# tzt101/MichiGAN

Measured on NVIDIA H100. Metric: 512x512 images/sec (generator forward), higher is better.
Workload: dtype fp16/bf16 tensor-core operands (bf16 hi+lo split where needed), fp32 accumulate and storage

## Files before the change

michigan_b200/csrc/mg_conv3x3.cu:

```cuda
#include <cuda.h>
#include <cuda_runtime.h>
#include <cstring>
#include <type_traits>
#include "mg_ptx.cuh"
#include "mg_internal.h"
#include "mg_epilogue.cuh"

namespace mg {

constexpr int kGM = 2;
constexpr int kPatchW = 8 * kGM + 2;
constexpr int kPatchH = 16 + 2;
constexpr int kPatchTx = kPatchW * kPatchH * 128;
constexpr int kPatchBytes = (kPatchTx + 1023) & ~1023;
constexpr int kMaxBSlots = 8;
constexpr int kASlots = 2;

struct Conv3Params {
    IgemmParams g;
    int groups_w, num_groups, b_slots, b_slot_bytes, steps_hi, steps_lo, n_items, bar3_off;
};

template <int FMT, int BN, bool MERGED, int SPEC, int CW, bool REG>
__global__ void __launch_bounds__(kThreads, 1)
conv3x3_group_kernel(const __grid_constant__ CUtensorMap tmA, const __grid_constant__ CUtensorMap tmA2,
                     const __grid_constant__ CUtensorMap tmB, const Conv3Params q) {
    constexpr int kAcc = MERGED ? 2 * BN : BN;
    const IgemmParams& p = q.g;
    extern __shared__ __align__(1024) uint8_t smem_raw[];
    uint8_t* smem = reinterpret_cast<uint8_t*>((reinterpret_cast<uintptr_t>(smem_raw) + 1023) & ~uintptr_t(1023));
    uint8_t* a_ring = smem;
    uint8_t* b_ring = smem + kASlots * kPatchBytes;
    uint64_t* bars = reinterpret_cast<uint64_t*>(smem + q.bar3_off);
    uint64_t* bfull = bars;
    uint64_t* bempty = bars + kMaxBSlots;
    uint64_t* afull = bars + 2 * kMaxBSlots;
    uint64_t* aempty = afull + kASlots;
    float* acc_tile = reinterpret_cast<float*>(smem + p.acc_off);

    const int warp = threadIdx.x >> 5;
    const int lane = threadIdx.x & 31;

    if (warp == kNumEpiWarps && lane == 0) {
        tma_prefetch_desc(&tmA);
        tma_prefetch_desc(&tmA2);
        tma_prefetch_desc(&tmB);
        for (int s = 0; s < q.b_slots; ++s) { mbar_init(&bfull[s], 1); mbar_init(&bempty[s], kNumEpiWarps); }
        for (int s = 0; s < kASlots; ++s) { mbar_init(&afull[s], 1); mbar_init(&aempty[s], kNumEpiWarps); }
        fence_barrier_init();
    }
    __syncthreads();
    const int groups_per_img = q.groups_w * p.tiles_h;
    const bool split = p.parts > 1;

    if (warp >= kNumEpiWarps) {
        setmaxnreg_dec<kProducerRegs>();
        if (warp == kNumEpiWarps && lane == 0) {
            int bs = 0, as_ = 0;
            uint32_t bph = 0, aphs = 0;
            int gia = blockIdx.x, ita = 0;
            long long a_issued = 0, item = 0;
            auto issue_a = [&](bool must) -> bool {
                if (gia >= q.num_groups) return false;
                if (!must && !mbar_test_wait(&aempty[as_], aphs ^ 1)) return false;
                if (must) mbar_wait_report(&aempty[as_], aphs ^ 1);
                const int mga = gia / p.n_tiles;
                const int gwa = mga % q.groups_w, tha = (mga / q.groups_w) % p.tiles_h, tna = mga / groups_per_img;
                const int kca = split ? (ita >> 1) : ita, parta = split ? (ita & 1) : 0;
                mbar_arrive_expect_tx(&afull[as_], (uint32_t)kPatchTx);
                tma_load_4d(a_ring + (size_t)as_ * kPatchBytes, parta ? &tmA2 : &tmA, &afull[as_], kca * p.kelem, gwa * (8 * kGM) - 1,
                            tha * 16 - 1, tna);
                if (++as_ == kASlots) { as_ = 0; aphs ^= 1; }
                if (++ita == q.n_items) { ita = 0; gia += gridDim.x; }
                ++a_issued;
                return true;
            };
            for (int gi = blockIdx.x; gi < q.num_groups; gi += gridDim.x) {
                const int nt = gi % p.n_tiles;
                for (int it = 0; it < q.n_items; ++it, ++item) {
                    const int kc = split ? (it >> 1) : it, part = split ? (it & 1) : 0;
                    if (a_issued <= item) issue_a(true);
                    const int steps = part ? q.steps_lo : q.steps_hi;
                    for (int st = 0; st < steps; ++st) {
                        if (a_issued < item + kASlots) issue_a(false);
                        int tap, wsel;
                        if (steps == 18) { tap = st >> 1; wsel = st & 1; } else { tap = st; wsel = 0; }
                        const int kofs = (split ? (tap * 2 + wsel) : tap) * p.Cin + kc * p.kelem;
                        mbar_wait_report(&bempty[bs], bph ^ 1);
                        uint8_t* sb = b_ring + (size_t)bs * q.b_slot_bytes;
                        if (p.merged && part == 0) {
                            mbar_arrive_expect_tx(&bfull[bs], (uint32_t)(2 * p.BN * 128));
                            tma_load_2d(sb, &tmB, &bfull[bs], kofs, nt * p.BN);
                            tma_load_2d(sb + p.BN * 128, &tmB, &bfull[bs], kofs + p.Cin, nt * p.BN);
                        } else {
                            mbar_arrive_expect_tx(&bfull[bs], (uint32_t)(p.BN * 128));
                            tma_load_2d(sb, &tmB, &bfull[bs], kofs, nt * p.BN);
                        }
                        if (++bs == q.b_slots) { bs = 0; bph ^= 1; }
                    }
                }
            }
        }
    } else {
        setmaxnreg_inc<kConsumerRegs>();
        const int wg = warp >> 2;
        const int quarter = warp & 3;
        const int half = warp >> 2;
        const uint32_t a_base0 = smem_u32(a_ring), b_base0 = smem_u32(b_ring);
        float acc0[kAcc / 2], acc1[kAcc / 2];
        int bs = 0, as_ = 0;
        uint32_t bph = 0, aphs = 0;
        int held_b = -1, held_a = -1;
        auto release_held = [&]() {
            __syncwarp();
            if (lane == 0) {
                if (held_b >= 0) mbar_arrive(&bempty[held_b]);
                if (held_a >= 0) mbar_arrive(&aempty[held_a]);
            }
            held_b = held_a = -1;
        };
        for (int gi = blockIdx.x; gi < q.num_groups; gi += gridDim.x) {
            const int nt = gi % p.n_tiles;
            const int mg = gi / p.n_tiles;
            const int gw = mg % q.groups_w, th = (mg / q.groups_w) % p.tiles_h, tn = mg / groups_per_img;
            for (int it = 0; it < q.n_items; ++it) {
                const int part = split ? (it & 1) : 0;
                mbar_wait(&afull[as_], aphs);
                const uint32_t a_base = a_base0 + (uint32_t)(as_ * kPatchBytes) + (uint32_t)(wg * 8 * kPatchW * 128);
                const int steps = part ? q.steps_lo : q.steps_hi;
                auto item = [&](auto n_cols) {
                    constexpr int N = decltype(n_cols)::value;
                    for (int st = 0; st < steps; ++st) {
                        const int tap = steps == 18 ? (st >> 1) : st;
                        const int kh = tap / 3, kw = tap - kh * 3;
                        mbar_wait(&bfull[bs], bph);
                        const uint32_t a_tap = a_base + (uint32_t)((kh * kPatchW + kw) * 128);
                        const uint64_t db = wg_desc_sw128(b_base0 + (uint32_t)(bs * q.b_slot_bytes), 1024);
                        wgmma_fence();
#pragma unroll
                        for (int k = 0; k < 4; ++k) {
                            const uint32_t accum = (it | st | k) != 0 ? 1u : 0u;
                            const uint64_t da0 = wg_desc_sw128(a_tap + (uint32_t)(k * 32), (uint32_t)(kPatchW * 128));
                            const uint64_t da1 = wg_desc_sw128(a_tap + (uint32_t)(8 * 128 + k * 32), (uint32_t)(kPatchW * 128));
                            wgmma_step<FMT, N>(acc0, da0, db + (uint64_t)(2 * k), accum);
                            wgmma_step<FMT, N>(acc1, da1, db + (uint64_t)(2 * k), accum);
                        }
                        wgmma_commit();
                        wgmma_wait<1>();
                        release_held();
                        held_b = bs;
                        if (++bs == q.b_slots) { bs = 0; bph ^= 1; }
                    }
                };
                if (MERGED && part == 1) item(std::integral_constant<int, BN>{});
                else item(std::integral_constant<int, kAcc>{});
                held_a = as_;
                if (++as_ == kASlots) { as_ = 0; aphs ^= 1; }
            }
            wgmma_wait<0>();
            wgmma_fence_operand(acc0);
            wgmma_fence_operand(acc1);
            release_held();
            if constexpr (REG) {
                epilogue_frag<SPEC, BN, MERGED>(p, acc0, acc1, nt, gw * kGM, th, tn, wg, quarter, lane);
            } else {
                float* scr = reinterpret_cast<float*>(smem + p.epi_off) + warp * (32 * (CW + 4));
                bar_sync(1, kNumEpiWarps * 32);
                acc_store(acc_tile, p.acc_ld, acc0, kAcc, wg * 64);
                bar_sync(1, kNumEpiWarps * 32);
                epilogue_tile<SPEC, CW>(p, scr, acc_tile, nt, gw * kGM, th, tn, quarter, half, lane);
                bar_sync(1, kNumEpiWarps * 32);
                acc_store(acc_tile, p.acc_ld, acc1, kAcc, wg * 64);
                bar_sync(1, kNumEpiWarps * 32);
                epilogue_tile<SPEC, CW>(p, scr, acc_tile, nt, gw * kGM + 1, th, tn, quarter, half, lane);
            }
        }
    }
}

constexpr bool conv3_reg_epilogue(int bn, bool merged, int spec) { return !(bn == 128 && !merged && spec == 0); }

struct Conv3Launch {
    const CUtensorMap *tmA, *tmA2, *tmB;
    const Conv3Params* q;
    int grid;
    size_t smem_bytes;
    cudaStream_t stream;
    bool reg;
    template <int FMT, int BN, bool MERGED, int SPEC, int CW>
    int run() const {
        if constexpr (conv_variant_exists<FMT, BN, MERGED, SPEC, CW>()) {
            if constexpr (CW == 16 && conv3_reg_epilogue(BN, MERGED, SPEC)) {
                if (reg) {
                    static thread_local int attr_dev_reg = -1;
                    return launch_conv_kernel(conv3x3_group_kernel<FMT, BN, MERGED, SPEC, CW, true>, attr_dev_reg, grid, smem_bytes,
                                              stream, *tmA, *tmA2, *tmB, *q);
                }
            }
            static thread_local int attr_dev = -1;
            return launch_conv_kernel(conv3x3_group_kernel<FMT, BN, MERGED, SPEC, CW, false>, attr_dev, grid, smem_bytes, stream, *tmA,
                                      *tmA2, *tmB, *q);
        } else {
            return set_error(-14, "conv3x3: no kernel variant for format %d, BN %d, merged %d, SPEC %d, CW %d", FMT, BN, (int)MERGED,
                             SPEC, CW);
        }
    }
};

int conv3x3_group_launch(const mg_igemm_args* a, IgemmParams& p, int BN, int cw, int scratch_bytes, int spec, cudaStream_t stream) {
    if (!(a->KH == 3 && a->KW == 3 && a->stride == 1 && p.pad_h == 1 && p.pad_w == 1 && a->H == a->OH && a->W == a->OW && p.epi_impl == 1 &&
          a->OW >= 16 && a->OW % 16 == 0 && a->OH >= 16 && p.os == 1))
        return 0;
    const bool reg = tune(TK_EPI_REG) != 0 && conv3_reg_epilogue(BN, p.merged != 0, spec);
    if (reg) { scratch_bytes = 0; cw = 16; }
    const int acc_bytes = reg ? 0 : 128 * p.acc_ld * 4;
    {
        const int avail0 = 227 * 1024 - 1024 - 512 - scratch_bytes - acc_bytes - kASlots * kPatchBytes;
        if (avail0 / (p.acc_cols * 128) < 3) return 0;
    }
    Conv3Params q;
    memset(&q, 0, sizeof(q));
    p.TW = 8; p.TH = 16; p.TN = 1;
    p.tiles_w = a->OW / 8;
    p.tiles_h = (a->OH + 15) / 16;
    p.tiles_n = a->N;
    p.num_tiles = p.tiles_w * p.tiles_h * p.tiles_n * p.n_tiles;
    p.halo = 0;
    q.groups_w = p.tiles_w / kGM;
    q.num_groups = q.groups_w * p.tiles_h * p.tiles_n * p.n_tiles;
    const bool split = a->split != 0;
    q.steps_hi = (split && !p.merged) ? 18 : 9;
    q.steps_lo = 9;
    q.n_items = p.kchunks * (split ? 2 : 1);
    q.b_slot_bytes = p.acc_cols * 128;
    const int avail = 227 * 1024 - 1024 - 512 - scratch_bytes - acc_bytes - kASlots * kPatchBytes;
    q.b_slots = avail / q.b_slot_bytes;
    if (q.b_slots > kMaxBSlots) q.b_slots = kMaxBSlots;
    const size_t ring_bytes = (size_t)kASlots * kPatchBytes + (size_t)q.b_slots * q.b_slot_bytes;
    q.bar3_off = (int)ring_bytes;
    p.epi_off = (int)ring_bytes + 512;
    p.acc_off = p.epi_off + scratch_bytes;
    p.parts = p.merged ? 2 : (split ? 3 : 1);
    q.g = p;

    CUtensorMap tmA, tmA2, tmB;
    const int kelem = p.kelem;
    const int esz = a->a_fmt == 0 ? 4 : 2;
    const CUtensorMapDataType dt = a->a_fmt == 0 ? CU_TENSOR_MAP_DATA_TYPE_FLOAT32
                                 : a->a_fmt == 1 ? CU_TENSOR_MAP_DATA_TYPE_FLOAT16 : CU_TENSOR_MAP_DATA_TYPE_BFLOAT16;
    {
        cuuint64_t dims[4] = {(cuuint64_t)a->Cin, (cuuint64_t)a->W, (cuuint64_t)a->H, (cuuint64_t)a->N};
        cuuint64_t strides[3] = {(cuuint64_t)a->Cin * esz, (cuuint64_t)a->W * a->Cin * esz, (cuuint64_t)a->H * a->W * a->Cin * esz};
        cuuint32_t box[4] = {(cuuint32_t)kelem, (cuuint32_t)kPatchW, (cuuint32_t)kPatchH, 1};
        cuuint32_t estr[4] = {1, 1, 1, 1};
        int rc = encode_tensor_map(&tmA, (void*)a->in, dt, 4, dims, strides, box, estr, CU_TENSOR_MAP_SWIZZLE_128B);
        if (rc) return rc;
        rc = encode_tensor_map(&tmA2, (void*)(split ? a->in_lo : a->in), dt, 4, dims, strides, box, estr, CU_TENSOR_MAP_SWIZZLE_128B);
        if (rc) return rc;
    }
    {
        const int coutg = a->epi == MG_EPI_SPADE ? 2 * a->Cout : a->Cout;
        const cuuint64_t ktot = (cuuint64_t)9 * a->Cin * (split ? 2 : 1);
        cuuint64_t dims[2] = {ktot, (cuuint64_t)coutg};
        cuuint64_t strides[1] = {ktot * esz};
        cuuint32_t box[2] = {(cuuint32_t)kelem, (cuuint32_t)BN};
        cuuint32_t estr[2] = {1, 1};
        int rc = encode_tensor_map(&tmB, (void*)a->wpack, dt, 2, dims, strides, box, estr, CU_TENSOR_MAP_SWIZZLE_128B);
        if (rc) return rc;
    }
    const size_t smem_bytes = ring_bytes + 1024 + 512 + scratch_bytes + acc_bytes;
    int grid = num_sms();
    if (a->max_ctas > 0 && a->max_ctas < grid) grid = a->max_ctas;
    if (grid > q.num_groups) grid = q.num_groups;
    const Conv3Launch l{&tmA, &tmA2, &tmB, &q, grid, smem_bytes, stream, reg};
    const int rc = dispatch_conv_variant(l, p.a_fmt, BN, p.merged != 0, spec, cw);
    return rc == 0 ? 1 : rc;
}

}
```

michigan_b200/csrc/mg_epilogue.cuh:

```cuda
#pragma once
#include <cuda.h>
#include <cuda_runtime.h>
#include <cuda_fp16.h>
#include <cuda_bf16.h>
#include <type_traits>
#include "mg_ptx.cuh"
#include "mg_internal.h"

namespace mg {

constexpr int kNumEpiWarps = 8;
constexpr int kThreads = kNumEpiWarps * 32 + 128;
constexpr int kProducerRegs = 40;
constexpr int kConsumerRegs = 232;
static_assert(kProducerRegs * 128 + kConsumerRegs * kNumEpiWarps * 32 <= 65536, "register split exceeds the SM's file");
constexpr int kMaxAccCols = 128;
constexpr int kABytes = 128 * 128;
constexpr int kMaxStages = 8;
constexpr int kMaxASlots = 4;

struct IgemmParams {
    int N, OH, OW, Cout;
    int Cin, KH, KW, stride, pad_h, pad_w;
    int os, ooh, oow, OHF, OWF, accumulate;
// ... 170 lines not shown
                m.z = epi_spade_mod(xv.z, sc4.z, sh4.z, g14.z, av[j].z, gs.z);
                m.w = epi_spade_mod(xv.w, sc4.w, sh4.w, g14.w, av[j].w, gs.w);
                if (has_aux) *reinterpret_cast<float4*>(p.aux + (size_t)pixo[j] * p.Cout + cch) = gs;
                av[j] = m;
            }
            if (p.merged) load_chunk(col + ch_tile + p.BN, bv, true);
        }
        if (!ch_ok) continue;
#pragma unroll
        for (int j = 0; j < passes; ++j) {
            if (!((vmask >> j) & 1u)) continue;
            const size_t pix = pixo[j];
            float y[4];
            if (spade) {
                y[0] = epi_spade_out(av[j].x, bb4.x, bv[j].x, act); y[1] = epi_spade_out(av[j].y, bb4.y, bv[j].y, act);
                y[2] = epi_spade_out(av[j].z, bb4.z, bv[j].z, act); y[3] = epi_spade_out(av[j].w, bb4.w, bv[j].w, act);
            } else {
                const float ps = p.pscale ? __ldg(p.pscale + pix) : 1.f;
                const bool has_res = p.res != nullptr;
                const float4 rv = has_res ? pre[j] : bias4;
                y[0] = epi_plain(av[j].x, ps, bias4.x, has_res, rv.x, act); y[1] = epi_plain(av[j].y, ps, bias4.y, has_res, rv.y, act);
                y[2] = epi_plain(av[j].z, ps, bias4.z, has_res, rv.z, act); y[3] = epi_plain(av[j].w, ps, bias4.w, has_res, rv.w, act);
                if (p.bf) {
                    const int rr = quarter * 32 + j * ppp + psub;
                    const size_t mp = ((size_t)(tn * p.TN + (rr >> (twl + thl))) * p.MH +
                                       (size_t)(th * p.TH + ((rr >> twl) & (p.TH - 1))) * p.mask_stride) * p.MW +
                                      (size_t)(tw * p.TW + (rr & (p.TW - 1))) * p.mask_stride;
                    const float om_hair = 1.f - __ldg(p.hair + mp), om_back = 1.f - __ldg(p.back + mp);
                    const float4 bfv = __ldg(reinterpret_cast<const float4*>(p.bf + pix * p.Cout + cch));
                    y[0] = epi_blend(y[0], bfv.x, om_hair, om_back); y[1] = epi_blend(y[1], bfv.y, om_hair, om_back);
                    y[2] = epi_blend(y[2], bfv.z, om_hair, om_back); y[3] = epi_blend(y[3], bfv.w, om_hair, om_back);
                }
                if (p.pmul) {
                    const float pm = __ldg(p.pmul + pix);
#pragma unroll
                    for (int i = 0; i < 4; ++i) y[i] = epi_pmul(y[i], pm);
                }
            }
            if (do_round) {
#pragma unroll
                for (int i = 0; i < 4; ++i) y[i] = round_tf32(y[i]);
            }
            if (has_out) {
                float4* op = reinterpret_cast<float4*>(p.out + pix * p.Cout + cch);
                if (p.accumulate) {
                    const float4 o = *op;
                    y[0] += o.x; y[1] += o.y; y[2] += o.z; y[3] += o.w;
                }
                *op = make_float4(y[0], y[1], y[2], y[3]);
            }
            if (has_hi && !((MG_DBGV(p) & (8 | 32)) && y[0] != 12345.f)) {
                uint32_t hi[2], lo[2];
#pragma unroll
                for (int i = 0; i < 2; ++i) epi_split16(y[2 * i], y[2 * i + 1], fmt16, hi[i], lo[i]);
                const size_t eo = pix * p.Cout + cch;
                *reinterpret_cast<uint2*>(reinterpret_cast<uint16_t*>(p.out_hi) + eo) = make_uint2(hi[0], hi[1]);
                if (has_lo) *reinterpret_cast<uint2*>(reinterpret_cast<uint16_t*>(p.out_lo) + eo) = make_uint2(lo[0], lo[1]);
            }
        }
    }
}

template <int SPEC>
__device__ __forceinline__ void epi_store_pair(const IgemmParams& p, size_t pix, int ch, float y0, float y1) {
    constexpr bool kS = SPEC == 1 || SPEC == 2;
    if (!kS && p.round_out != 0) { y0 = round_tf32(y0); y1 = round_tf32(y1); }
    const size_t eo = pix * p.Cout + ch;
    if (!kS && p.out != nullptr) {
        float2* op = reinterpret_cast<float2*>(p.out + eo);
        if (p.accumulate) {
            const float2 o = *op;
            y0 += o.x; y1 += o.y;
        }
        *op = make_float2(y0, y1);
    }
    if ((kS || p.out_hi != nullptr) && !((MG_DBGV(p) & (8 | 32)) && y0 != 12345.f)) {
        uint32_t hi, lo;
        epi_split16(y0, y1, kS ? 2 : p.out16_fmt, hi, lo);
        *reinterpret_cast<uint32_t*>(reinterpret_cast<uint16_t*>(p.out_hi) + eo) = hi;
        if (kS || p.out_lo != nullptr) *reinterpret_cast<uint32_t*>(reinterpret_cast<uint16_t*>(p.out_lo) + eo) = lo;
    }
}

template <int SPEC, int BN, bool MERGED, int R>
__device__ __forceinline__ void epilogue_frag(const IgemmParams& p, const float (&acc0)[R], const float (&acc1)[R], int nt, int tw0,
                                              int th, int tn, int wg, int quarter, int lane) {
    constexpr bool kS = SPEC == 1 || SPEC == 2;
    constexpr int kLo = BN / 8;
    static_assert(R == (MERGED ? BN : BN / 2), "accumulator registers: 64 x N per warpgroup is N / 2 per thread");
    const int act = SPEC == 1 ? 2 : (SPEC == 2 ? 0 : p.act);
    if (MG_DBGV(p) & 4) return;
    const int c0 = 2 * (lane & 3);
    size_t pix[2][2], src[2][2];
    bool ok[2][2];
#pragma unroll
    for (int t = 0; t < 2; ++t)
#pragma unroll
        for (int h = 0; h < 2; ++h) {
            const int ow = (tw0 + t) * 8 + (lane >> 2), oh = th * 16 + 8 * wg + 2 * quarter + h, n = tn;
            ok[t][h] = ow < p.OW && oh < p.OH;
            pix[t][h] = ((size_t)n * p.OHF + (size_t)oh + p.ooh) * p.OWF + (size_t)ow + p.oow;
            if (kS || p.epi == 1) src[t][h] = ((size_t)n * p.XH + (oh >> p.x_shift)) * p.XW + (ow >> p.x_shift);
            else src[t][h] = ((size_t)n * p.RH + (oh >> p.res_shift)) * p.RW + (ow >> p.res_shift);
        }
    const bool side_ok = !(MG_DBGV(p) & (8 | 64));

    if constexpr (BN % 64 == 0) {
        if (kS || p.epi == 1) {
            constexpr int J = BN / 16, kBeta = BN / 16;
            const int ch0 = nt * (BN / 2) + c0;
            const bool has_aux = !kS && p.aux != nullptr;
            float2 xv[2][2][J];
            auto load_x = [&](auto tc) {
                constexpr int t = decltype(tc)::value;
#pragma unroll
                for (int h = 0; h < 2; ++h)
#pragma unroll
                    for (int j = 0; j < J; ++j)
                        xv[t][h][j] = ok[t][h] && side_ok && ch0 + 8 * j < p.Cout
                                          ? __ldg(reinterpret_cast<const float2*>(p.x + src[t][h] * p.Cout + ch0 + 8 * j))
                                          : make_float2(0.f, 0.f);
            };
            auto tile = [&](const float (&acc)[R], auto tc) {
                constexpr int t = decltype(tc)::value;
#pragma unroll
                for (int j = 0; j < J; ++j) {
                    const int ch = ch0 + 8 * j;
                    if (ch >= p.Cout) continue;
                    const float2 sc = __ldg(reinterpret_cast<const float2*>(p.nscale + ch));
                    const float2 sh = __ldg(reinterpret_cast<const float2*>(p.nshift + ch));
                    const float2 g1 = __ldg(reinterpret_cast<const float2*>(p.gbias1 + ch));
                    const float2 bb = __ldg(reinterpret_cast<const float2*>(p.bbias + ch));
#pragma unroll
                    for (int h = 0; h < 2; ++h) {
                        if (!ok[t][h]) continue;
                        const float2 x = side_ok ? xv[t][h][j] : sc;
                        float g[2], b[2], gs[2], y[2];
#pragma unroll
                        for (int e = 0; e < 2; ++e) {
                            g[e] = acc[4 * j + 2 * h + e];
                            b[e] = acc[4 * (j + kBeta) + 2 * h + e];
                            if (MERGED) {
                                g[e] += acc[4 * (j + kLo) + 2 * h + e];
                                b[e] += acc[4 * (j + kBeta + kLo) + 2 * h + e];
                            }
                        }
                        y[0] = epi_spade_out(epi_spade_mod(x.x, sc.x, sh.x, g1.x, g[0], gs[0]), bb.x, b[0], act);
                        y[1] = epi_spade_out(epi_spade_mod(x.y, sc.y, sh.y, g1.y, g[1], gs[1]), bb.y, b[1], act);
                        if (has_aux) *reinterpret_cast<float2*>(p.aux + pix[t][h] * p.Cout + ch) = make_float2(gs[0], gs[1]);
                        epi_store_pair<SPEC>(p, pix[t][h], ch, y[0], y[1]);
                    }
                }
            };
            load_x(std::integral_constant<int, 0>{});
            if constexpr (kS) load_x(std::integral_constant<int, 1>{});
            tile(acc0, std::integral_constant<int, 0>{});
            if constexpr (!kS) load_x(std::integral_constant<int, 1>{});
            tile(acc1, std::integral_constant<int, 1>{});
            return;
        }
    }
    if constexpr (!kS) {
        constexpr int J = BN / 8;
        const int ch0 = nt * BN + c0;
        const bool has_res = p.res != nullptr, has_bf = p.bf != nullptr;
        auto row = [&](const float (&acc)[R], auto tc, auto hc) {
            constexpr int t = decltype(tc)::value, h = decltype(hc)::value;
            if (!ok[t][h]) return;
            float2 rv[J], bfv[J];
            const float ps = p.pscale ? __ldg(p.pscale + pix[t][h]) : 1.f;
            const float pm = p.pmul ? __ldg(p.pmul + pix[t][h]) : 1.f;
            float om_hair = 0.f, om_back = 0.f;
            if (has_bf) {
                const int ow = (tw0 + t) * 8 + (lane >> 2), oh = th * 16 + 8 * wg + 2 * quarter + h;
                const size_t mp = ((size_t)tn * p.MH + (size_t)oh * p.mask_stride) * p.MW + (size_t)ow * p.mask_stride;
                om_hair = 1.f - __ldg(p.hair + mp);
                om_back = 1.f - __ldg(p.back + mp);
            }
#pragma unroll
            for (int j = 0; j < J; ++j) {
                const bool cok = ch0 + 8 * j < p.Cout;
                rv[j] = cok && has_res && side_ok ? __ldg(reinterpret_cast<const float2*>(p.res + src[t][h] * p.Cout + ch0 + 8 * j))
                                                  : make_float2(0.f, 0.f);
                bfv[j] = cok && has_bf ? __ldg(reinterpret_cast<const float2*>(p.bf + pix[t][h] * p.Cout + ch0 + 8 * j))
                                       : make_float2(0.f, 0.f);
            }
#pragma unroll
            for (int j = 0; j < J; ++j) {
                const int ch = ch0 + 8 * j;
                if (ch >= p.Cout) continue;
                const float2 bias = p.bias ? __ldg(reinterpret_cast<const float2*>(p.bias + ch)) : make_float2(0.f, 0.f);
                float a[2], y[2];
#pragma unroll
                for (int e = 0; e < 2; ++e) {
                    a[e] = acc[4 * j + 2 * h + e];
                    if (MERGED) a[e] += acc[4 * (j + kLo) + 2 * h + e];
                }
                y[0] = epi_plain(a[0], ps, bias.x, has_res, rv[j].x, act);
                y[1] = epi_plain(a[1], ps, bias.y, has_res, rv[j].y, act);
                if (has_bf) {
                    y[0] = epi_blend(y[0], bfv[j].x, om_hair, om_back);
                    y[1] = epi_blend(y[1], bfv[j].y, om_hair, om_back);
                }
                if (p.pmul) { y[0] = epi_pmul(y[0], pm); y[1] = epi_pmul(y[1], pm); }
                epi_store_pair<SPEC>(p, pix[t][h], ch, y[0], y[1]);
            }
        };
        using I0 = std::integral_constant<int, 0>;
        using I1 = std::integral_constant<int, 1>;
        row(acc0, I0{}, I0{});
        row(acc0, I0{}, I1{});
        row(acc1, I1{}, I0{});
        row(acc1, I1{}, I1{});
    }
}

template <int FMT, int BN, bool MERGED, int SPEC, int CW>
constexpr bool conv_variant_exists() {
    return (!MERGED || (FMT != 0 && 2 * BN <= kMaxAccCols)) && (SPEC == 0 || BN % 64 == 0) &&
           (CW == 16 || (SPEC == 0 ? BN >= 64 : BN == 128));
}

template <int FMT, int BN, bool MERGED, int SPEC, class L>
int dispatch_cw(const L& l, int cw) {
    if (cw == 16) return l.template run<FMT, BN, MERGED, SPEC, 16>();
    if (cw == 32) return l.template run<FMT, BN, MERGED, SPEC, 32>();
    return set_error(-14, "conv kernel: no variant for epilogue chunk width %d", cw);
}
template <int FMT, int BN, bool MERGED, class L>
int dispatch_spec(const L& l, int spec, int cw) {
    if (spec == 0) return dispatch_cw<FMT, BN, MERGED, 0>(l, cw);
    if (spec == 1) return dispatch_cw<FMT, BN, MERGED, 1>(l, cw);
    if (spec == 2) return dispatch_cw<FMT, BN, MERGED, 2>(l, cw);
    return set_error(-14, "conv kernel: no variant for epilogue specialisation %d", spec);
}
template <int FMT, int BN, class L>
int dispatch_merged(const L& l, bool merged, int spec, int cw) {
    return merged ? dispatch_spec<FMT, BN, true>(l, spec, cw) : dispatch_spec<FMT, BN, false>(l, spec, cw);
// ... 34 lines not shown
```

michigan_b200/csrc/mg_ptx.cuh:

```cuda
#pragma once
#include <cstdint>
#include <cstdio>
#include <cuda_runtime.h>

namespace mg {

__device__ __forceinline__ uint32_t smem_u32(const void* p) {
    return static_cast<uint32_t>(__cvta_generic_to_shared(p));
}

__device__ __forceinline__ bool elect_one() {
    uint32_t pred;
    asm volatile(
        "{\n\t.reg .pred P;\n\t"
        "elect.sync _|P, 0xffffffff;\n\t"
        "selp.u32 %0, 1, 0, P;\n\t}\n"
        : "=r"(pred));
    return pred != 0;
}

__device__ __forceinline__ void mbar_init(uint64_t* bar, uint32_t count) {
    asm volatile("mbarrier.init.shared::cta.b64 [%0], %1;\n" ::"r"(smem_u32(bar)), "r"(count));
}
__device__ __forceinline__ void fence_barrier_init() {
    asm volatile("fence.mbarrier_init.release.cluster;\n" ::: "memory");
}
__device__ __forceinline__ void fence_proxy_async_smem() {
    asm volatile("fence.proxy.async.shared::cta;\n" ::: "memory");
}
__device__ __forceinline__ void mbar_arrive_expect_tx(uint64_t* bar, uint32_t bytes) {
    asm volatile("mbarrier.arrive.expect_tx.shared::cta.b64 _, [%0], %1;\n" ::"r"(smem_u32(bar)),
                 "r"(bytes)
                 : "memory");
}
__device__ __forceinline__ void mbar_arrive(uint64_t* bar) {
    asm volatile("mbarrier.arrive.shared::cta.b64 _, [%0];\n" ::"r"(smem_u32(bar)) : "memory");
}
__device__ __forceinline__ bool mbar_try_wait(uint64_t* bar, uint32_t parity) {
    uint32_t ok;
    asm volatile(
        "{\n\t.reg .pred P;\n\t"
        "mbarrier.try_wait.parity.shared::cta.b64 P, [%1], %2;\n\t"
        "selp.u32 %0, 1, 0, P;\n\t}\n"
        : "=r"(ok)
        : "r"(smem_u32(bar)), "r"(parity)
        : "memory");
    return ok != 0;
}
__device__ __forceinline__ bool mbar_test_wait(uint64_t* bar, uint32_t parity) {
    uint32_t ok;
    asm volatile(
        "{\n\t.reg .pred P;\n\t"
        "mbarrier.test_wait.parity.shared::cta.b64 P, [%1], %2;\n\t"
        "selp.u32 %0, 1, 0, P;\n\t}\n"
        : "=r"(ok)
        : "r"(smem_u32(bar)), "r"(parity)
        : "memory");
    return ok != 0;
}
#ifndef MG_SPIN_LIMIT
#define MG_SPIN_LIMIT (1u << 26)
#endif
__device__ __forceinline__ void mbar_wait(uint64_t* bar, uint32_t parity) {
    uint32_t spins = 0;
    while (!mbar_try_wait(bar, parity)) {
        if (++spins > MG_SPIN_LIMIT) __trap();
    }
}
__device__ __forceinline__ void mbar_wait_report(uint64_t* bar, uint32_t parity) {
    uint32_t spins = 0;
    while (!mbar_try_wait(bar, parity)) {
        if (++spins > MG_SPIN_LIMIT) {
#ifdef MG_WAIT_PRINTF
            printf("mg: mbarrier timeout blk %d thr %d bar %p parity %u\n", blockIdx.x, threadIdx.x, (void*)bar, parity);
#endif
            __trap();
        }
    }
}

__device__ __forceinline__ void tma_prefetch_desc(const void* tmap) {
    asm volatile("prefetch.tensormap [%0];\n" ::"l"(tmap) : "memory");
}
__device__ __forceinline__ void tma_load_2d(void* dst, const void* tmap, uint64_t* bar, int c0, int c1) {
    asm volatile(
        "cp.async.bulk.tensor.2d.shared::cluster.global.tile.mbarrier::complete_tx::bytes"
        " [%0], [%1, {%3, %4}], [%2];\n" ::"r"(smem_u32(dst)),
        "l"(tmap), "r"(smem_u32(bar)), "r"(c0), "r"(c1)
        : "memory");
}
__device__ __forceinline__ void tma_load_4d(void* dst, const void* tmap, uint64_t* bar, int c0, int c1,
                                            int c2, int c3) {
    asm volatile(
        "cp.async.bulk.tensor.4d.shared::cluster.global.tile.mbarrier::complete_tx::bytes"
        " [%0], [%1, {%3, %4, %5, %6}], [%2];\n" ::"r"(smem_u32(dst)),
        "l"(tmap), "r"(smem_u32(bar)), "r"(c0), "r"(c1), "r"(c2), "r"(c3)
        : "memory");
}
__device__ __forceinline__ void tma_store_4d(const void* tmap, const void* src, int c0, int c1, int c2, int c3) {
    asm volatile("cp.async.bulk.tensor.4d.global.shared::cta.tile.bulk_group [%0, {%2, %3, %4, %5}], [%1];"
                 :: "l"(tmap), "r"(smem_u32(src)), "r"(c0), "r"(c1), "r"(c2), "r"(c3) : "memory");
}
__device__ __forceinline__ void tma_store_commit() { asm volatile("cp.async.bulk.commit_group;" ::: "memory"); }
__device__ __forceinline__ void tma_store_wait_read() { asm volatile("cp.async.bulk.wait_group.read 0;" ::: "memory"); }
__device__ __forceinline__ void tma_store_wait_all() { asm volatile("cp.async.bulk.wait_group 0;" ::: "memory"); }

__device__ __forceinline__ void tma_load_3d(void* dst, const void* tmap, uint64_t* bar, int c0, int c1,
                                            int c2) {
    asm volatile(
        "cp.async.bulk.tensor.3d.shared::cluster.global.tile.mbarrier::complete_tx::bytes"
        " [%0], [%1, {%3, %4, %5}], [%2];\n" ::"r"(smem_u32(dst)),
        "l"(tmap), "r"(smem_u32(bar)), "r"(c0), "r"(c1), "r"(c2)
        : "memory");
}

__device__ __forceinline__ void wgmma_fence() { asm volatile("wgmma.fence.sync.aligned;\n" ::: "memory"); }
__device__ __forceinline__ void wgmma_commit() { asm volatile("wgmma.commit_group.sync.aligned;\n" ::: "memory"); }
__device__ __forceinline__ void wgmma_wait_all() { asm volatile("wgmma.wait_group.sync.aligned 0;\n" ::: "memory"); }
template <int N>
__device__ __forceinline__ void wgmma_wait() { asm volatile("wgmma.wait_group.sync.aligned %0;\n" ::"n"(N) : "memory"); }
template <int R>
__device__ __forceinline__ void wgmma_fence_operand(float (&acc)[R]) {
#pragma unroll
    for (int i = 0; i < R; ++i) asm volatile("" : "+f"(acc[i])::"memory");
}
template <int R>
__device__ __forceinline__ void setmaxnreg_dec() { asm volatile("setmaxnreg.dec.sync.aligned.u32 %0;\n" ::"n"(R)); }
template <int R>
__device__ __forceinline__ void setmaxnreg_inc() { asm volatile("setmaxnreg.inc.sync.aligned.u32 %0;\n" ::"n"(R)); }
__device__ __forceinline__ void bar_sync(int id, int count) {
    asm volatile("bar.sync %0, %1;\n" ::"r"(id), "r"(count) : "memory");
}

__device__ __forceinline__ uint64_t wg_desc_sw128(uint32_t smem_addr, uint32_t sbo_bytes) {
    uint64_t d = 0;
    d |= (uint64_t)((smem_addr & 0x3FFFF) >> 4);
    d |= (uint64_t)1 << 16;
    d |= (uint64_t)((sbo_bytes >> 4) & 0x3FFF) << 32;
    d |= (uint64_t)1 << 62;
    return d;
}

__device__ __forceinline__ void wgmma_tf32_n32(float (&d)[16], uint64_t da, uint64_t db, uint32_t scale_d) {
    asm volatile(
        "{\n\t.reg .pred p;\n\tsetp.ne.b32 p, %18, 0;\n\t"
        "wgmma.mma_async.sync.aligned.m64n32k8.f32.tf32.tf32 {%0, %1, %2, %3, %4, %5, %6, %7, %8, %9, %10, %11, %12, %13, %14, %15}, %16, %17, p, 1, 1;\n\t}\n"
        : "+f"(d[0]), "+f"(d[1]), "+f"(d[2]), "+f"(d[3]), "+f"(d[4]), "+f"(d[5]), "+f"(d[6]), "+f"(d[7]), "+f"(d[8]), "+f"(d[9]), "+f"(d[10]), "+f"(d[11]), "+f"(d[12]), "+f"(d[13]), "+f"(d[14]), "+f"(d[15])
        : "l"(da), "l"(db), "r"(scale_d));
}
__device__ __forceinline__ void wgmma_f16_n32(float (&d)[16], uint64_t da, uint64_t db, uint32_t scale_d) {
    asm volatile(
        "{\n\t.reg .pred p;\n\tsetp.ne.b32 p, %18, 0;\n\t"
        "wgmma.mma_async.sync.aligned.m64n32k16.f32.f16.f16 {%0, %1, %2, %3, %4, %5, %6, %7, %8, %9, %10, %11, %12, %13, %14, %15}, %16, %17, p, 1, 1, 0, 0;\n\t}\n"
        : "+f"(d[0]), "+f"(d[1]), "+f"(d[2]), "+f"(d[3]), "+f"(d[4]), "+f"(d[5]), "+f"(d[6]), "+f"(d[7]), "+f"(d[8]), "+f"(d[9]), "+f"(d[10]), "+f"(d[11]), "+f"(d[12]), "+f"(d[13]), "+f"(d[14]), "+f"(d[15])
        : "l"(da), "l"(db), "r"(scale_d));
}
__device__ __forceinline__ void wgmma_bf16_n32(float (&d)[16], uint64_t da, uint64_t db, uint32_t scale_d) {
    asm volatile(
        "{\n\t.reg .pred p;\n\tsetp.ne.b32 p, %18, 0;\n\t"
        "wgmma.mma_async.sync.aligned.m64n32k16.f32.bf16.bf16 {%0, %1, %2, %3, %4, %5, %6, %7, %8, %9, %10, %11, %12, %13, %14, %15}, %16, %17, p, 1, 1, 0, 0;\n\t}\n"
        : "+f"(d[0]), "+f"(d[1]), "+f"(d[2]), "+f"(d[3]), "+f"(d[4]), "+f"(d[5]), "+f"(d[6]), "+f"(d[7]), "+f"(d[8]), "+f"(d[9]), "+f"(d[10]), "+f"(d[11]), "+f"(d[12]), "+f"(d[13]), "+f"(d[14]), "+f"(d[15])
        : "l"(da), "l"(db), "r"(scale_d));
}
__device__ __forceinline__ void wgmma_tf32_n64(float (&d)[32], uint64_t da, uint64_t db, uint32_t scale_d) {
    asm volatile(
        "{\n\t.reg .pred p;\n\tsetp.ne.b32 p, %34, 0;\n\t"
        "wgmma.mma_async.sync.aligned.m64n64k8.f32.tf32.tf32 {%0, %1, %2, %3, %4, %5, %6, %7, %8, %9, %10, %11, %12, %13, %14, %15, %16, %17, %18, %19, %20, %21, %22, %23, %24, %25, %26, %27, %28, %29, %30, %31}, %32, %33, p, 1, 1;\n\t}\n"
        : "+f"(d[0]), "+f"(d[1]), "+f"(d[2]), "+f"(d[3]), "+f"(d[4]), "+f"(d[5]), "+f"(d[6]), "+f"(d[7]), "+f"(d[8]), "+f"(d[9]), "+f"(d[10]), "+f"(d[11]), "+f"(d[12]), "+f"(d[13]), "+f"(d[14]), "+f"(d[15]), "+f"(d[16]), "+f"(d[17]), "+f"(d[18]), "+f"(d[19]), "+f"(d[20]), "+f"(d[21]), "+f"(d[22]), "+f"(d[23]), "+f"(d[24]), "+f"(d[25]), "+f"(d[26]), "+f"(d[27]), "+f"(d[28]), "+f"(d[29]), "+f"(d[30]), "+f"(d[31])
        : "l"(da), "l"(db), "r"(scale_d));
}
__device__ __forceinline__ void wgmma_f16_n64(float (&d)[32], uint64_t da, uint64_t db, uint32_t scale_d) {
    asm volatile(
        "{\n\t.reg .pred p;\n\tsetp.ne.b32 p, %34, 0;\n\t"
        "wgmma.mma_async.sync.aligned.m64n64k16.f32.f16.f16 {%0, %1, %2, %3, %4, %5, %6, %7, %8, %9, %10, %11, %12, %13, %14, %15, %16, %17, %18, %19, %20, %21, %22, %23, %24, %25, %26, %27, %28, %29, %30, %31}, %32, %33, p, 1, 1, 0, 0;\n\t}\n"
        : "+f"(d[0]), "+f"(d[1]), "+f"(d[2]), "+f"(d[3]), "+f"(d[4]), "+f"(d[5]), "+f"(d[6]), "+f"(d[7]), "+f"(d[8]), "+f"(d[9]), "+f"(d[10]), "+f"(d[11]), "+f"(d[12]), "+f"(d[13]), "+f"(d[14]), "+f"(d[15]), "+f"(d[16]), "+f"(d[17]), "+f"(d[18]), "+f"(d[19]), "+f"(d[20]), "+f"(d[21]), "+f"(d[22]), "+f"(d[23]), "+f"(d[24]), "+f"(d[25]), "+f"(d[26]), "+f"(d[27]), "+f"(d[28]), "+f"(d[29]), "+f"(d[30]), "+f"(d[31])
        : "l"(da), "l"(db), "r"(scale_d));
}
__device__ __forceinline__ void wgmma_bf16_n64(float (&d)[32], uint64_t da, uint64_t db, uint32_t scale_d) {
    asm volatile(
        "{\n\t.reg .pred p;\n\tsetp.ne.b32 p, %34, 0;\n\t"
        "wgmma.mma_async.sync.aligned.m64n64k16.f32.bf16.bf16 {%0, %1, %2, %3, %4, %5, %6, %7, %8, %9, %10, %11, %12, %13, %14, %15, %16, %17, %18, %19, %20, %21, %22, %23, %24, %25, %26, %27, %28, %29, %30, %31}, %32, %33, p, 1, 1, 0, 0;\n\t}\n"
        : "+f"(d[0]), "+f"(d[1]), "+f"(d[2]), "+f"(d[3]), "+f"(d[4]), "+f"(d[5]), "+f"(d[6]), "+f"(d[7]), "+f"(d[8]), "+f"(d[9]), "+f"(d[10]), "+f"(d[11]), "+f"(d[12]), "+f"(d[13]), "+f"(d[14]), "+f"(d[15]), "+f"(d[16]), "+f"(d[17]), "+f"(d[18]), "+f"(d[19]), "+f"(d[20]), "+f"(d[21]), "+f"(d[22]), "+f"(d[23]), "+f"(d[24]), "+f"(d[25]), "+f"(d[26]), "+f"(d[27]), "+f"(d[28]), "+f"(d[29]), "+f"(d[30]), "+f"(d[31])
        : "l"(da), "l"(db), "r"(scale_d));
}
__device__ __forceinline__ void wgmma_tf32_n128(float (&d)[64], uint64_t da, uint64_t db, uint32_t scale_d) {
    asm volatile(
        "{\n\t.reg .pred p;\n\tsetp.ne.b32 p, %66, 0;\n\t"
        "wgmma.mma_async.sync.aligned.m64n128k8.f32.tf32.tf32 {%0, %1, %2, %3, %4, %5, %6, %7, %8, %9, %10, %11, %12, %13, %14, %15, %16, %17, %18, %19, %20, %21, %22, %23, %24, %25, %26, %27, %28, %29, %30, %31, %32, %33, %34, %35, %36, %37, %38, %39, %40, %41, %42, %43, %44, %45, %46, %47, %48, %49, %50, %51, %52, %53, %54, %55, %56, %57, %58, %59, %60, %61, %62, %63}, %64, %65, p, 1, 1;\n\t}\n"
// ... 92 lines not shown
```

Before: 160.4.

## Stage SPADE conv epilogue outputs in swizzled smem and write via TMA stores

For the SPADE register-epilogue variants, the bf16 hi/lo outputs are written into a per-warp swizzled shared-memory stage and sent to global memory with 4D TMA bulk stores, replacing per-thread global stores. The producer also issues L2 prefetches of the residual/x tile for each group, and the second warpgroup is held back a few steps behind the first so the two epilogues do not collide. This reduces scattered global store traffic and epilogue latency, at the cost of extra shared memory (fewer B pipeline slots), extra barriers, and dropping the aux store on that path.

New measurement: 163.7 (median of 6 runs). 2.1% higher.

```diff
diff --git a/michigan_b200/csrc/mg_conv3x3.cu b/michigan_b200/csrc/mg_conv3x3.cu
--- a/michigan_b200/csrc/mg_conv3x3.cu
+++ b/michigan_b200/csrc/mg_conv3x3.cu
@@ -15,17 +15,24 @@
 constexpr int kPatchBytes = (kPatchTx + 1023) & ~1023;
 constexpr int kMaxBSlots = 8;
 constexpr int kASlots = 2;
+constexpr int kStageWarpBytes = 4096;
+
+__host__ __device__ constexpr bool conv3_tma_store(int spec) { return spec == 1 || spec == 2; }
+__host__ __device__ constexpr int conv3_lag(bool reg, int spec) { return reg && conv3_tma_store(spec) ? 4 : 0; }
 
 struct Conv3Params {
     IgemmParams g;
-    int groups_w, num_groups, b_slots, b_slot_bytes, steps_hi, steps_lo, n_items, bar3_off;
+    int groups_w, num_groups, b_slots, b_slot_bytes, steps_hi, steps_lo, n_items, bar3_off, stage_off;
 };
 
 template <int FMT, int BN, bool MERGED, int SPEC, int CW, bool REG>
 __global__ void __launch_bounds__(kThreads, 1)
 conv3x3_group_kernel(const __grid_constant__ CUtensorMap tmA, const __grid_constant__ CUtensorMap tmA2,
-                     const __grid_constant__ CUtensorMap tmB, const Conv3Params q) {
+                     const __grid_constant__ CUtensorMap tmB, const __grid_constant__ CUtensorMap tmO,
+                     const __grid_constant__ CUtensorMap tmO2, const __grid_constant__ CUtensorMap tmX, const Conv3Params q) {
     constexpr int kAcc = MERGED ? 2 * BN : BN;
+    constexpr bool kTmaStore = REG && conv3_tma_store(SPEC);
+    constexpr int kLag = conv3_lag(REG, SPEC);
     const IgemmParams& p = q.g;
     extern __shared__ __align__(1024) uint8_t smem_raw[];
     uint8_t* smem = reinterpret_cast<uint8_t*>((reinterpret_cast<uintptr_t>(smem_raw) + 1023) & ~uintptr_t(1023));
@@ -36,6 +43,7 @@
     uint64_t* bempty = bars + kMaxBSlots;
     uint64_t* afull = bars + 2 * kMaxBSlots;
     uint64_t* aempty = afull + kASlots;
+    uint64_t* lead = aempty + kASlots;
     float* acc_tile = reinterpret_cast<float*>(smem + p.acc_off);
 
     const int warp = threadIdx.x >> 5;
@@ -45,8 +53,10 @@
         tma_prefetch_desc(&tmA);
         tma_prefetch_desc(&tmA2);
         tma_prefetch_desc(&tmB);
+        if (kTmaStore) { tma_prefetch_desc(&tmO); tma_prefetch_desc(&tmO2); tma_prefetch_desc(&tmX); }
         for (int s = 0; s < q.b_slots; ++s) { mbar_init(&bfull[s], 1); mbar_init(&bempty[s], kNumEpiWarps); }
         for (int s = 0; s < kASlots; ++s) { mbar_init(&afull[s], 1); mbar_init(&aempty[s], kNumEpiWarps); }
+        mbar_init(lead, kNumEpiWarps / 2);
         fence_barrier_init();
     }
     __syncthreads();
@@ -70,6 +80,9 @@
                 mbar_arrive_expect_tx(&afull[as_], (uint32_t)kPatchTx);
                 tma_load_4d(a_ring + (size_t)as_ * kPatchBytes, parta ? &tmA2 : &tmA, &afull[as_], kca * p.kelem, gwa * (8 * kGM) - 1,
                             tha * 16 - 1, tna);
+                if (kTmaStore && ita == q.n_items - 1) {
+                    tma_prefetch_l2_4d(&tmX, (gia % p.n_tiles) * (p.BN / 2), (gwa * 16) >> p.x_shift, (tha * 16) >> p.x_shift, tna);
+                }
                 if (++as_ == kASlots) { as_ = 0; aphs ^= 1; }
                 if (++ita == q.n_items) { ita = 0; gia += gridDim.x; }
                 ++a_issued;
@@ -119,6 +132,7 @@
             }
             held_b = held_a = -1;
         };
+        if (kLag > 0 && wg == 1) mbar_wait(lead, 0);
         for (int gi = blockIdx.x; gi < q.num_groups; gi += gridDim.x) {
             const int nt = gi % p.n_tiles;
             const int mg = gi / p.n_tiles;
@@ -150,6 +164,7 @@
                         release_held();
                         held_b = bs;
                         if (++bs == q.b_slots) { bs = 0; bph ^= 1; }
+                        if (kLag > 0 && wg == 0 && lane == 0 && gi == (int)blockIdx.x && it == 0 && st == kLag - 1) mbar_arrive(lead);
                     }
                 };
                 if (MERGED && part == 1) item(std::integral_constant<int, BN>{});
@@ -162,7 +177,9 @@
             wgmma_fence_operand(acc1);
             release_held();
             if constexpr (REG) {
-                epilogue_frag<SPEC, BN, MERGED>(p, acc0, acc1, nt, gw * kGM, th, tn, wg, quarter, lane);
+                uint8_t* stage = kTmaStore ? smem + q.stage_off + warp * kStageWarpBytes : nullptr;
+                epilogue_frag<SPEC, BN, MERGED>(p, acc0, acc1, nt, gw * kGM, th, tn, wg, quarter, lane, stage, &tmO, &tmO2);
+                if (kTmaStore && gi + (int)gridDim.x >= q.num_groups) tma_store_wait_all();
             } else {
                 float* scr = reinterpret_cast<float*>(smem + p.epi_off) + warp * (32 * (CW + 4));
                 bar_sync(1, kNumEpiWarps * 32);
@@ -181,7 +198,7 @@
 constexpr bool conv3_reg_epilogue(int bn, bool merged, int spec) { return !(bn == 128 && !merged && spec == 0); }
 
 struct Conv3Launch {
-    const CUtensorMap *tmA, *tmA2, *tmB;
+    const CUtensorMap *tmA, *tmA2, *tmB, *tmO, *tmO2, *tmX;
     const Conv3Params* q;
     int grid;
     size_t smem_bytes;
@@ -194,12 +211,12 @@
                 if (reg) {
                     static thread_local int attr_dev_reg = -1;
                     return launch_conv_kernel(conv3x3_group_kernel<FMT, BN, MERGED, SPEC, CW, true>, attr_dev_reg, grid, smem_bytes,
-                                              stream, *tmA, *tmA2, *tmB, *q);
+                                              stream, *tmA, *tmA2, *tmB, *tmO, *tmO2, *tmX, *q);
                 }
             }
             static thread_local int attr_dev = -1;
             return launch_conv_kernel(conv3x3_group_kernel<FMT, BN, MERGED, SPEC, CW, false>, attr_dev, grid, smem_bytes, stream, *tmA,
-                                      *tmA2, *tmB, *q);
+                                      *tmA2, *tmB, *tmO, *tmO2, *tmX, *q);
         } else {
             return set_error(-14, "conv3x3: no kernel variant for format %d, BN %d, merged %d, SPEC %d, CW %d", FMT, BN, (int)MERGED,
                              SPEC, CW);
@@ -214,9 +231,13 @@
     const bool reg = tune(TK_EPI_REG) != 0 && conv3_reg_epilogue(BN, p.merged != 0, spec);
     if (reg) { scratch_bytes = 0; cw = 16; }
     const int acc_bytes = reg ? 0 : 128 * p.acc_ld * 4;
+    const bool tma_store = reg && conv3_tma_store(spec);
+    if (tma_store && (a->Cout % 8 != 0 || ((uintptr_t)a->out_hi | (uintptr_t)a->out_lo | (uintptr_t)a->x) % 16 != 0)) return 0;
+    const int stage_bytes = tma_store ? kNumEpiWarps * kStageWarpBytes : 0;
+    const int lag = reg ? conv3_lag(true, spec) : 0;
     {
-        const int avail0 = 227 * 1024 - 1024 - 512 - scratch_bytes - acc_bytes - kASlots * kPatchBytes;
-        if (avail0 / (p.acc_cols * 128) < 3) return 0;
+        const int avail0 = 227 * 1024 - 1024 - 512 - scratch_bytes - acc_bytes - stage_bytes - kASlots * kPatchBytes;
+        if (avail0 / (p.acc_cols * 128) < (lag > 0 ? lag + 2 : 3)) return 0;
     }
     Conv3Params q;
     memset(&q, 0, sizeof(q));
@@ -233,12 +254,13 @@
     q.steps_lo = 9;
     q.n_items = p.kchunks * (split ? 2 : 1);
     q.b_slot_bytes = p.acc_cols * 128;
-    const int avail = 227 * 1024 - 1024 - 512 - scratch_bytes - acc_bytes - kASlots * kPatchBytes;
+    const int avail = 227 * 1024 - 1024 - 512 - scratch_bytes - acc_bytes - stage_bytes - kASlots * kPatchBytes;
     q.b_slots = avail / q.b_slot_bytes;
     if (q.b_slots > kMaxBSlots) q.b_slots = kMaxBSlots;
     const size_t ring_bytes = (size_t)kASlots * kPatchBytes + (size_t)q.b_slots * q.b_slot_bytes;
-    q.bar3_off = (int)ring_bytes;
-    p.epi_off = (int)ring_bytes + 512;
+    q.stage_off = (int)ring_bytes;
+    q.bar3_off = (int)ring_bytes + stage_bytes;
+    p.epi_off = q.bar3_off + 512;
     p.acc_off = p.epi_off + scratch_bytes;
     p.parts = p.merged ? 2 : (split ? 3 : 1);
     q.g = p;
@@ -268,11 +290,33 @@
         int rc = encode_tensor_map(&tmB, (void*)a->wpack, dt, 2, dims, strides, box, estr, CU_TENSOR_MAP_SWIZZLE_128B);
         if (rc) return rc;
     }
-    const size_t smem_bytes = ring_bytes + 1024 + 512 + scratch_bytes + acc_bytes;
+    CUtensorMap tmO, tmO2, tmX;
+    memset(&tmO, 0, sizeof(tmO));
+    memset(&tmO2, 0, sizeof(tmO2));
+    memset(&tmX, 0, sizeof(tmX));
+    if (tma_store) {
+        cuuint64_t dims[4] = {(cuuint64_t)a->Cout, (cuuint64_t)p.OWF, (cuuint64_t)p.OHF, (cuuint64_t)a->N};
+        cuuint64_t strides[3] = {(cuuint64_t)a->Cout * 2, (cuuint64_t)p.OWF * a->Cout * 2, (cuuint64_t)p.OHF * p.OWF * a->Cout * 2};
+        cuuint32_t box[4] = {(cuuint32_t)(BN / 2), 8, 2, 1};
+        cuuint32_t estr[4] = {1, 1, 1, 1};
+        const CUtensorMapSwizzle sw = BN == 128 ? CU_TENSOR_MAP_SWIZZLE_128B : CU_TENSOR_MAP_SWIZZLE_64B;
+        int rc = encode_tensor_map(&tmO, a->out_hi, CU_TENSOR_MAP_DATA_TYPE_BFLOAT16, 4, dims, strides, box, estr, sw);
+        if (rc) return rc;
+        rc = encode_tensor_map(&tmO2, a->out_lo, CU_TENSOR_MAP_DATA_TYPE_BFLOAT16, 4, dims, strides, box, estr, sw);
+        if (rc) return rc;
+        cuuint64_t xdims[4] = {(cuuint64_t)a->Cout, (cuuint64_t)p.XW, (cuuint64_t)p.XH, (cuuint64_t)a->N};
+        cuuint64_t xstrides[3] = {(cuuint64_t)a->Cout * 4, (cuuint64_t)p.XW * a->Cout * 4, (cuuint64_t)p.XH * p.XW * a->Cout * 4};
+        cuuint32_t xbox[4] = {(cuuint32_t)(BN / 2), (cuuint32_t)(p.x_shift < 4 ? 16 >> p.x_shift : 1),
+                            (cuuint32_t)(p.x_shift < 4 ? 16 >> p.x_shift : 1), 1};
+        rc = encode_tensor_map(&tmX, (void*)a->x, CU_TENSOR_MAP_DATA_TYPE_FLOAT32, 4, xdims, xstrides, xbox, estr,
+                               CU_TENSOR_MAP_SWIZZLE_NONE);
+        if (rc) return rc;
+    }
+    const size_t smem_bytes = ring_bytes + stage_bytes + 1024 + 512 + scratch_bytes + acc_bytes;
     int grid = num_sms();
     if (a->max_ctas > 0 && a->max_ctas < grid) grid = a->max_ctas;
     if (grid > q.num_groups) grid = q.num_groups;
-    const Conv3Launch l{&tmA, &tmA2, &tmB, &q, grid, smem_bytes, stream, reg};
+    const Conv3Launch l{&tmA, &tmA2, &tmB, &tmO, &tmO2, &tmX, &q, grid, smem_bytes, stream, reg};
     const int rc = dispatch_conv_variant(l, p.a_fmt, BN, p.merged != 0, spec, cw);
     return rc == 0 ? 1 : rc;
 }
diff --git a/michigan_b200/csrc/mg_epilogue.cuh b/michigan_b200/csrc/mg_epilogue.cuh
--- a/michigan_b200/csrc/mg_epilogue.cuh
+++ b/michigan_b200/csrc/mg_epilogue.cuh
@@ -276,9 +276,14 @@
     }
 }
 
+template <int BN>
+__device__ __forceinline__ uint32_t stage_swizzle(uint32_t off) {
+    return BN == 128 ? off ^ (((off >> 7) & 7u) << 4) : off ^ (((off >> 7) & 3u) << 4);
+}
 template <int SPEC, int BN, bool MERGED, int R>
 __device__ __forceinline__ void epilogue_frag(const IgemmParams& p, const float (&acc0)[R], const float (&acc1)[R], int nt, int tw0,
-                                              int th, int tn, int wg, int quarter, int lane) {
+                                              int th, int tn, int wg, int quarter, int lane, uint8_t* stage, const CUtensorMap* tmO,
+                                              const CUtensorMap* tmO2) {
     constexpr bool kS = SPEC == 1 || SPEC == 2;
     constexpr int kLo = BN / 8;
     static_assert(R == (MERGED ? BN : BN / 2), "accumulator registers: 64 x N per warpgroup is N / 2 per thread");
@@ -317,6 +322,11 @@
             };
             auto tile = [&](const float (&acc)[R], auto tc) {
                 constexpr int t = decltype(tc)::value;
+                const uint32_t stage_s = smem_u32(stage);
+                if constexpr (kS) {
+                    if (lane == 0) tma_store_wait_read();
+                    __syncwarp();
+                }
 #pragma unroll
                 for (int j = 0; j < J; ++j) {
                     const int ch = ch0 + 8 * j;
@@ -341,13 +351,31 @@
                         }
                         y[0] = epi_spade_out(epi_spade_mod(x.x, sc.x, sh.x, g1.x, g[0], gs[0]), bb.x, b[0], act);
                         y[1] = epi_spade_out(epi_spade_mod(x.y, sc.y, sh.y, g1.y, g[1], gs[1]), bb.y, b[1], act);
-                        if (has_aux) *reinterpret_cast<float2*>(p.aux + pix[t][h] * p.Cout + ch) = make_float2(gs[0], gs[1]);
-                        epi_store_pair<SPEC>(p, pix[t][h], ch, y[0], y[1]);
+                        if constexpr (kS) {
+                            uint32_t hi, lo;
+                            epi_split16(y[0], y[1], 2, hi, lo);
+                            const uint32_t o = stage_swizzle<BN>((uint32_t)((h * 8 + (lane >> 2)) * BN + 16 * j + 2 * c0));
+                            st_shared_u32(stage_s + o, hi);
+                            st_shared_u32(stage_s + 2048 + o, lo);
+                        } else {
+                            if (has_aux) *reinterpret_cast<float2*>(p.aux + pix[t][h] * p.Cout + ch) = make_float2(gs[0], gs[1]);
+                            epi_store_pair<SPEC>(p, pix[t][h], ch, y[0], y[1]);
+                        }
+                    }
+                }
+                if constexpr (kS) {
+                    if constexpr (t == 0) load_x(std::integral_constant<int, 1>{});
+                    fence_proxy_async_smem();
+                    __syncwarp();
+                    if (lane == 0 && !(MG_DBGV(p) & (8 | 32))) {
+                        const int ow = (tw0 + t) * 8 + p.oow, oh = th * 16 + 8 * wg + 2 * quarter + p.ooh;
+                        tma_store_4d(tmO, stage, nt * (BN / 2), ow, oh, tn);
+                        tma_store_4d(tmO2, stage + 2048, nt * (BN / 2), ow, oh, tn);
+                        tma_store_commit();
                     }
                 }
             };
             load_x(std::integral_constant<int, 0>{});
-            if constexpr (kS) load_x(std::integral_constant<int, 1>{});
             tile(acc0, std::integral_constant<int, 0>{});
             if constexpr (!kS) load_x(std::integral_constant<int, 1>{});
             tile(acc1, std::integral_constant<int, 1>{});
diff --git a/michigan_b200/csrc/mg_ptx.cuh b/michigan_b200/csrc/mg_ptx.cuh
--- a/michigan_b200/csrc/mg_ptx.cuh
+++ b/michigan_b200/csrc/mg_ptx.cuh
@@ -17,6 +17,10 @@
         "selp.u32 %0, 1, 0, P;\n\t}\n"
         : "=r"(pred));
     return pred != 0;
+}
+
+__device__ __forceinline__ void st_shared_u32(uint32_t addr, uint32_t v) {
+    asm volatile("st.shared.b32 [%0], %1;\n" ::"r"(addr), "r"(v));
 }
 
 __device__ __forceinline__ void mbar_init(uint64_t* bar, uint32_t count) {
@@ -104,6 +108,11 @@
 __device__ __forceinline__ void tma_store_commit() { asm volatile("cp.async.bulk.commit_group;" ::: "memory"); }
 __device__ __forceinline__ void tma_store_wait_read() { asm volatile("cp.async.bulk.wait_group.read 0;" ::: "memory"); }
 __device__ __forceinline__ void tma_store_wait_all() { asm volatile("cp.async.bulk.wait_group 0;" ::: "memory"); }
+
+__device__ __forceinline__ void tma_prefetch_l2_4d(const void* tmap, int c0, int c1, int c2, int c3) {
+    asm volatile("cp.async.bulk.prefetch.tensor.4d.L2.global.tile [%0, {%1, %2, %3, %4}];"
+                 :: "l"(tmap), "r"(c0), "r"(c1), "r"(c2), "r"(c3) : "memory");
+}
 
 __device__ __forceinline__ void tma_load_3d(void* dst, const void* tmap, uint64_t* bar, int c0, int c1,
                                             int c2) {
```
